# Psy-Fer/SquiggleKit

Measured on AMD Instinct MI355X. Metric: reads/sec MotifSeq DTW (4k-sample read x 200-sample motif), higher is better.
Workload: dtype f64 results; u32 fixed-point screening

## Files before the change

squigglekit_amd/csrc/sk_common.h:

```cpp
#pragma once
#include <hip/hip_runtime.h>
#include <stdint.h>
#include <stddef.h>
#include <stdarg.h>
#include <vector>
#include "squigglekit_hip.h"

#define SK_MAX_DEVICES 16
#define SK_WAVE 64

struct sk_prep {
    int32_t n;
    int32_t flags;
    double  center;
    double  scale;
    double  top;
    double  bot;
};

#define SK_IFLAG_INPLACE 0x100
#define SK_FLAG_PUBLIC   0xff

enum sk_prep_mode { SK_PREP_MEDMAD = 0, SK_PREP_ZSCALE = 1, SK_PREP_SEGMENT = 2, SK_PREP_DRNA = 3 };

// ... 76 lines not shown
    std::vector<int32_t> panel_long;
    sk_buf ckpt;
    sk_buf motifq;
    sk_buf motif64;
    bool   motif64_valid = false;
    std::vector<double> motif64_host;
    sk_buf lastq;
    sk_buf qflag;
    sk_buf wsoft;
    sk_buf lsum;
    sk_buf wstate;
    sk_buf wrec;
    sk_buf wrecq;
    sk_buf order;
    sk_buf motifw;
    std::vector<double> motifw_host;
    int    motifq_L = 0;
    sk_buf retry;
    sk_buf dtwcnt;
    sk_buf audit;
    sk_buf sib;
    sk_buf sibout;
    sk_buf sibstate;
    bool   retry_dev = false;
    std::vector<unsigned> motifq_host;
    bool   motifq_valid = false;
    sk_buf redo;
    int    redo_route = SK_REDO_NONE;
    std::vector<size_t> redo_off;
    size_t redo_used = 0;
    std::vector<int64_t> pa_off_host;
    int    last_retry = 0;
    std::vector<hipEvent_t> evpool;
    int    prof_chunks = 0;
    int    prof_reads[64] = {0};
    std::vector<double> motif_host;
    std::vector<double> motif_src;
    int    motif_L = 0;
    void  *comm = nullptr;
    void  *sessions[SK_STREAM_MAX_SESSIONS] = {};
    sk_buf commbuf;
};

const char *sk_tune(const char *name);

struct sk_entry {
// ... 75 lines not shown
int sk_launch_row_background(sk_ctx *c, const double *rowD, int64_t row_stride, const sk_hit *rec, int32_t nreads,
                             sk_bg_rec *out);
struct sk_path_args {
    int            feed;
    const void    *samples;
    const void    *samples_raw = nullptr;
    int64_t        stride = 0;
    const int64_t *off = nullptr;
    const sk_prep *prep = nullptr;
    int32_t        nreads = 0;
    int64_t        max_len = 0;
    const double  *d_motif = nullptr;
    int32_t        nmotif = 0;
    const sk_hit  *hits = nullptr;
    int32_t        K = 1;
    int32_t       *spans = nullptr;
};
int sk_path_begin(sk_ctx *c);
int sk_launch_paths(sk_ctx *c, const sk_path_args *p);
int sk_launch_events(sk_ctx *c, const sk_path_args *p, sk_event *events);
int sk_launch_events_pool(sk_ctx *c, const sk_event *d_ev, const uint8_t *d_use, int64_t nhits, int32_t N,
                          int32_t *d_idx, int32_t *d_cnt, sk_pool_rec *d_out);
int sk_launch_sdtw_screen(sk_ctx *c, const sk_sdtw_args *a, int ck, int span, int span2,
                          int32_t *d_retry_cnt, int32_t *d_retry, int32_t *d_early_cnt, int32_t *d_early);

__host__ __device__ static inline void sk_slice_indices(int32_t len, int32_t begin, int32_t end, int32_t *lo, int32_t *hi, int *clamped = nullptr)
{
    int64_t s = begin, e = end;
    int cl = 0;
    if (s < 0) { s += len; if (s < 0) { s = 0; cl |= 1; } } else if (s > len) { s = len; cl |= 1; }
    if (e < 0) { e += len; if (e < 0) { e = 0; cl |= 2; } } else if (e > len) { e = len; cl |= 2; }
    *lo = (int32_t)s; *hi = (int32_t)e;
    if (clamped) *clamped = cl;
}
int sk_launch_region_rows_i16(sk_ctx *c, const int16_t *d_sig, int64_t stride, const int32_t *d_len, int32_t nreads,
                              int32_t begin, int32_t end, const int32_t *d_win, int16_t *d_rows, int64_t wstride,
                              int32_t *d_wlen, int32_t *d_from);
int sk_launch_region_rows_f64(sk_ctx *c, const double *d_sig, const int64_t *d_src, const int64_t *d_woff, int32_t nreads,
                              double *d_out);
int sk_panel_plan(sk_ctx *c, const double *motifs, const int32_t *motif_off, int32_t nmotifs, const double *mean,
                  const double *sd, int64_t pairs);
int sk_launch_panel_dtw(sk_ctx *c, const sk_sdtw_args *base, const double *motifs, const int32_t *motif_off,
                        sk_hit *d_all, int64_t out_stride);
int sk_launch_panel_rank(sk_ctx *c, const sk_hit *d_all, int64_t out_stride, int32_t nreads, int32_t nmotifs,
                         sk_panel_rec *d_out);

struct sk_roll_params;
// ... 120 lines not shown
```

squigglekit_amd/csrc/sk_runtime.hip:

```cpp
#include "sk_common.h"
#include <string>
#include <string.h>
#include <mutex>
#include <stdio.h>
#include <stdlib.h>
#include <string.h>

static thread_local char  g_err[512] = "";
static thread_local int   g_cur = -1;
static sk_ctx             g_ctx[SK_MAX_DEVICES];
static std::mutex         g_mu;
static std::recursive_mutex g_ctx_mu[SK_MAX_DEVICES];

int sk_fail(int code, const char *fmt, ...)
{
    va_list ap;
    va_start(ap, fmt);
    vsnprintf(g_err, sizeof g_err, fmt, ap);
    va_end(ap);
    return code;
}

sk_entry::sk_entry() : sk_entry(g_cur) {}

// ... 37 lines not shown
{
    if (!c->stream2) {
        SK_HIP(hipStreamCreateWithFlags(&c->stream2, hipStreamNonBlocking));
        for (int i = 0; i < 9; i++) SK_HIP(hipEventCreateWithFlags(&c->ev_chunk[i], hipEventDisableTiming));
    }
    return SK_OK;
}

struct sk_tunable { const char *name, *test_values, *what; };
static const sk_tunable SK_TUNABLES[] = {
    {"SK_DTW_SCHEME",         "full exact2", "DTW scheme: full = one exact pass, exact2 = two exact passes (default: fixed-point screening + certified window)"},
    {"SK_DTW_QL",             "8 16 64",     "lanes per read of the screening scheme (default: by motif length and batch size)"},
    {"SK_DTW_NOFUSE",         "1",           "filter + medmad as their own kernel instead of the screening pass's prologue"},
    {"SK_DTW_FORCE_RETRY_PM", "100 1000",    "per-mille of reads sent through the exact retry whatever the window pass certified (sensitivity runs)"},
    {"SK_DTW_SPAN",           "150 300",     "look-back of the window pass in columns (one tier)"},
    {"SK_DTW_SPAN2",          "0 500",       "look-back of the window pass's second tier (0: none)"},
    {"SK_DTW_CK",             "64 256",      "steps between checkpoints of the screening pass (multiple of 64)"},
    {"SK_DTW_NOSORT",         "1",           "window passes take the reads in file order"},
    {"SK_DTW_NOHINT",         "1",           "no start hint: the plain screening sweep, every read's exact window looks back the same number of columns"},
    {"SK_DTW_HINT_MIN",       "1",           "the start hint is on for calls of at least this many reads (default 500000)"},
    {"SK_DTW_SORT_MIN",       "1",           "window passes sort chunks of at least this many reads"},
    {"SK_DTW_NO_EARLY",       "1",           "no early exact retry beside the window passes"},
    {"SK_DTW_NO_SIBLINGS",    "1",           "reads whose candidate columns fall into two clusters take the exact pass (no second window)"},
    {"SK_DTW_NOGUARD",        "1",           "screening scheme without its run-time guard (premise test in the window pass, audit, gated exact fallback): A/B cost runs"},
    {"SK_DTW_AUDIT_PERIOD",   "0 1 64",      "the audit re-runs one read in this many with the exact pass (default 4096; 0: no audit)"},
    {"SK_DTW_HOLE",           "qerr1 fma64 fma64x", "tests: a known precision hole put back (E = 1; the fma sample image for float64 reads, with / without the image-error guard) -- the guard has to notice and the records must not change"},
    {"SK_DTW_SCRATCH_MB",     "8 64",        "checkpoint scratch budget in MB (small values force many chunks)"},
    {"SK_DTW_NO_SMALL",       "1",           "small batches keep the batch lane layout"},
    {"SK_DTW_SMALL_MAX",      "0 100000",    "largest batch that spreads a read over 64 lanes"},
    {"SK_PREP_BLOCK",         "1",           "medmad statistics by the workgroup-per-read kernel"},
    {"SK_PREP_ROUNDS",        "1 3",         "grid rounds of the persistent statistics kernels"},
    {"SK_PREP_PERCU",         "1 2",         "workgroups per CU of the persistent statistics kernels"},
    {"SK_SEG_OLD",            "1",           "segmenter: numpy-order statistics kernels for every read"},
    {"SK_SEG_DELTA_SCALE",    "1e13",        "segmenter: certification margin multiplier (large: every read takes the numpy-order redo)"},
    {"SK_SEG_PA_F64",         "1",           "segmenter, raw reads through the pA conversion: expand to float64 and take the float64 kernels instead of the raw-domain kernel"},
    {"SK_SEG_NO_WG",          "1",           "segmenter, reads of 4 097 .. 65 536 samples: the wavefront-per-read statistics kernel (two looks at a read) instead of the workgroup-per-read one"},
    {"SK_SEG_WG_ALL",         "1",           "segmenter: the workgroup-per-read statistics kernel for every row of 4 097 .. 65 536 samples (default: where it is faster)"},
    {"SK_SEG_OCC",            "7 8",         "segmenter statistics kernel: waves per SIMD the registers are sized for"},
    {"SK_SEG_CHUNKS",         "2 8",         "segmenter: chunks of a large batch (walk of one beside the statistics of the next)"},
    {"SK_WALK_GENERAL",       "1",           "segmenter walk: general step (corrector test live)"},
    {"SK_WALK_SYNC",          "1",           "segmenter walk: run hopping with the 64 lanes of a wavefront on the same word (k_seg_walk3)"},
    {"SK_WALK_OWNPASS",       "1",           "segmenter walk: finds the quiet stretches and anchors in a pass of its own instead of taking the statistics kernel's hints"},
    {"SK_WALK_NOJUMP",        "1",           "segmenter walk: every run is hopped through, no jumps between the stretches of quiet entries"},
    {"SK_WALK_NOWAVE",        "1",           "segmenter walk: a lane per read also for long rows / small batches (no wavefront-per-read walk)"},
    {"SK_WALK_WAVE_MAXREADS", "0 1000000",   "segmenter walk: batches of up to this many reads take the wavefront-per-read walk (default: 16384, 131072 for rows beyond 4 096 samples)"},
    {"SK_DRNA_STEP",          "1",           "dRNA_segmenter, both branches: the per-sample scans instead of the scans by runs / by transitions"},
// ... 87 lines not shown
        c->num_cu = prop.multiProcessorCount;
        SK_HIP(hipStreamCreateWithFlags(&c->stream, hipStreamNonBlocking));
        for (int i = 0; i < 4; i++) SK_HIP(hipEventCreate(&c->ev[i]));
        c->ready = true;
    }
    g_cur = slot;
    return SK_OK;
}

static void free_buf(sk_buf *b) { if (b->p) (void)hipFree(b->p); b->p = nullptr; b->cap = 0; }

int sk_shutdown(void)
{
    std::lock_guard<std::mutex> lk(g_mu);
    for (int d = 0; d < SK_MAX_DEVICES; d++) {
        sk_ctx *c = &g_ctx[d];
        std::lock_guard<std::recursive_mutex> c_lock(g_ctx_mu[d]);
        if (!c->ready) continue;
        (void)hipSetDevice(c->device);
        (void)hipStreamSynchronize(c->stream);
        sk_stream_close_all(c);
        sk_buf *bufs[] = {&c->sig, &c->len, &c->off, &c->comp, &c->prep, &c->mask,
                          &c->motif, &c->out, &c->out2, &c->misc, &c->ckpt, &c->retry, &c->motifq, &c->lastq, &c->qflag,
                          &c->motif64, &c->commbuf, &c->dtwcnt, &c->wsoft, &c->wstate, &c->wrec, &c->motifw, &c->lsum, &c->wrecq, &c->order, &c->pacal, &c->seghints, &c->audit, &c->rlen, &c->redo, &c->sib, &c->sibout, &c->sibstate, &c->pull, &c->pulltext, &c->sweep, &c->sweeprec, &c->hitrows, &c->bgrec, &c->pathcnt, &c->pathlist, &c->pathscratch, &c->pathmotif, &c->pathspans, &c->events, &c->poolev, &c->pool, &c->panel, &c->panelwin, &c->panelaux, &c->panelrec, &c->seglev, &c->seglevwork, &c->detect, &c->detectout, &c->hmm, &c->hmmpath, &c->hmmseg};
        for (sk_buf *b : bufs) free_buf(b);
        for (int i = 0; i < 4; i++) (void)hipEventDestroy(c->ev[i]);
        for (hipEvent_t e : c->evpool) (void)hipEventDestroy(e);
        if (c->stream2) {
            (void)hipStreamSynchronize(c->stream2);
            for (int i = 0; i < 9; i++) if (c->ev_chunk[i]) (void)hipEventDestroy(c->ev_chunk[i]);
            (void)hipStreamDestroy(c->stream2);
        }
        if (c->stream3) {
            (void)hipStreamSynchronize(c->stream3);
            for (int i = 0; i < 2; i++) if (c->ev_r[i]) (void)hipEventDestroy(c->ev_r[i]);
            (void)hipStreamDestroy(c->stream3);
        }
        for (int i = 0; i < 2; i++) if (c->ev_s[i]) (void)hipEventDestroy(c->ev_s[i]);
        if (c->stream4) {
            (void)hipStreamSynchronize(c->stream4);
            if (c->ev_a) (void)hipEventDestroy(c->ev_a);
            (void)hipStreamDestroy(c->stream4);
        }
        (void)hipStreamDestroy(c->stream);
        *c = sk_ctx();
    }
    g_cur = -1;
// ... 180 lines not shown
```

squigglekit_amd/csrc/sk_sdtw.hip:

```cpp
#include "sk_sdtw_dev.h"
#include <math.h>
#include <stdlib.h>
#include <string.h>
#include <vector>

namespace {

template <int L, int R, int FEED, int MODE>
__global__ __launch_bounds__(256)
void k_sdtw(const sdtw_kargs a)
{
    static_assert(L == 16 || L == 64, "lanes per read");
    constexpr int G = 64 / L;
    constexpr int SHR = (L == 16) ? DPP_ROW_SHR1 : DPP_WAVE_SHR1;
    constexpr int ROL = (L == 16) ? DPP_ROW_ROL1 : DPP_WAVE_ROL1;
    constexpr bool TRACK = (MODE != MODE_DIST);
    constexpr int CKW = R + 3;
    const double INF = __builtin_huge_val();

    const int lane = threadIdx.x & 63;
    const int wave = blockIdx.x * (blockDim.x >> 6) + (threadIdx.x >> 6);
    const int g = lane / L, l = lane % L;
    int slot = wave * G + g;
    int nreads = a.nreads;
// ... 230 lines not shown
    if (s == 0) { list[0] = naudit; list[1] = 0; }
    if (s >= naudit) return;
    const int64_t base = (int64_t)s * period;
    const int span = (int)min((int64_t)period, (int64_t)nreads - base);
    unsigned h = (unsigned)s * 2654435761u + 0x9E3779B9u;
    h ^= salt * 0x9E3779B9u;
    h ^= h >> 15; h *= 0x85EBCA6Bu; h ^= h >> 13;
    list[2 + s] = (int)(base + (int64_t)(h % (unsigned)span));
}

__global__ void k_audit_compare(const int32_t *list, const sk_hit *exact, sk_hit *out, int naudit, int32_t *guard)
{
    const int s = blockIdx.x * blockDim.x + threadIdx.x;
    if (s >= naudit) return;
    const int r = list[2 + s];
    const sk_hit e = exact[s], g = out[r];
    const bool same_d = (__double_as_longlong(e.dist) == __double_as_longlong(g.dist)) || (e.dist != e.dist && g.dist != g.dist);
    if (same_d && e.start == g.start && e.end == g.end && e.n == g.n) return;
    out[r] = e;
    atomicAdd(&guard[SK_GUARD_MISMATCH], 1);
    atomicAdd(&guard[SK_GUARD_ALARM], 1);
}

static void sk_audit_pick(int32_t *list, int naudit, int period, int nreads, unsigned salt, hipStream_t st)
{
    hipLaunchKernelGGL(k_audit_pick, dim3((naudit + 255) / 256), dim3(256), 0, st, list, naudit, period, nreads, salt);
}
static void sk_audit_compare(const int32_t *list, const sk_hit *exact, sk_hit *out, int naudit, int32_t *guard, hipStream_t st)
{
    hipLaunchKernelGGL(k_audit_compare, dim3((naudit + 255) / 256), dim3(256), 0, st, list, exact, out, naudit, guard);
}

typedef void (*sdtw_fn)(const sdtw_kargs);

template <int L, int FEED, int MODE>
sdtw_fn pick_r(int R)
{
#define SK_KERNEL(RR) k_sdtw<L, RR, FEED, MODE>
    switch (R) { SK_R_CASES_1_16(SK_KERNEL) }
#undef SK_KERNEL
    return nullptr;
}

template <int FEED>
sdtw_fn pick(int L, int R, int mode)
{
// ... 251 lines not shown
    if (const char *e = sk_tune("SK_DTW_SCHEME")) qok = qok && strcmp(e, "exact2") != 0;
    int rc;
    if ((rc = sk_reserve(c, &c->retry, 2 * ((size_t)a->nreads + 2) * sizeof(int32_t)))) return rc;
    if ((rc = sk_reserve(c, &c->dtwcnt, 128))) return rc;
    int32_t *cnt = (int32_t *)c->retry.p;
    int32_t *ecnt = cnt + a->nreads + 2;
    SK_HIP(hipMemsetAsync(cnt, 0, sizeof(int32_t), c->stream));
    SK_HIP(hipMemsetAsync(ecnt, 0, sizeof(int32_t), c->stream));
    if (!a->accumulate) SK_HIP(hipMemsetAsync(c->dtwcnt.p, 0, 128, c->stream));
    c->retry_dev = true;
    if (L == 16 && !c->motif64_valid && pick_any(a->feed, 64, (N + 63) / 64, MODE_FULL)) {
        const int R64 = (N + 63) / 64;
        SK_HIP(hipStreamSynchronize(c->stream));
        if (c->stream3) SK_HIP(hipStreamSynchronize(c->stream3));
        if (c->stream4) SK_HIP(hipStreamSynchronize(c->stream4));
        c->motif64_host.resize((size_t)64 * R64);
        if (!sk_lane_layout(a->motif, N, 64, R64, c->motif64_host.data()))
            return sk_fail(SK_ERR_INVALID, "internal: motif layout mismatch");
        if ((rc = sk_reserve(c, &c->motif64, c->motif64_host.size() * sizeof(double)))) return rc;
        SK_HIP(hipMemcpyAsync(c->motif64.p, c->motif64_host.data(),
                              c->motif64_host.size() * sizeof(double), hipMemcpyHostToDevice, c->stream));
        c->motif64_valid = true;
    }
    auto launch_retry = [&](int32_t *list = nullptr, hipStream_t stream = nullptr) -> int {
        if (!list) list = cnt;
        sdtw_kargs kr = k;
        kr.read0 = 0; kr.ridx = list + 2; kr.count_ptr = list; kr.ckpt = nullptr;
        kr.total_ptr = (int32_t *)c->dtwcnt.p; kr.list_off = 0;
        const int R64 = (N + 63) / 64, P64 = 64 * R64 - N;
        sdtw_fn f64 = (L == 16) ? pick_any(a->feed, 64, R64, MODE_FULL) : nullptr;
        if (f64) {
            sdtw_kargs k64 = kr;
            k64.xlay = (const double *)c->motif64.p; k64.P = P64;
            k64.nreads = a->nreads < 8192 ? a->nreads : 8192;
            int rc2;
            if ((rc2 = launch(c, f64, k64, 64, stream))) return rc2;
            if (a->nreads <= 8192) return SK_OK;
            kr.list_off = 8192; kr.total_ptr = nullptr; kr.nreads = a->nreads - 8192;
            return launch(c, ff, kr, L, stream);
        }
        kr.nreads = a->nreads;
        return launch(c, ff, kr, L, stream);
    };
    if (a->fuse && !qok) return sk_fail(SK_ERR_INVALID, "internal: fused prologue without a screening pass");
    int32_t *guard = (int32_t *)c->dtwcnt.p + 8;
    const bool guarded = qok && sk_tune("SK_DTW_NOGUARD") == nullptr;
    int audit_period = 4096;
    if (const char *e = sk_tune("SK_DTW_AUDIT_PERIOD")) { const int v = atoi(e); if (v >= 0) audit_period = v; }
    int naudit = (guarded && audit_period > 0) ? (int)((a->nreads + audit_period - 1) / audit_period) : 0;
    if (naudit && sk_tune("SK_DTW_AUDIT_PERIOD") == nullptr) {
        const double audit_ms = (double)(maxlen + 64) * (8.0 * ((N + 63) / 64) + 20.0) * 5.0 / 2.4e6;
        const double window_ms = (double)a->nreads * N * 5.85e-8;
        const double call_ms = (double)a->nreads * (double)maxlen * N * 7.4e-11;
        const double exposed = audit_ms - window_ms;
        if (exposed > 0.02 * call_ms) {
            double kd = exposed / (0.02 * call_ms + 1e-9);
            const uint32_t K = kd > 64.0 ? 64u : (uint32_t)kd + 1u;
            if (c->dtw_sparse_calls++ % K) naudit = 0;
        }
    }
    int32_t *alist = nullptr;  sk_hit *aout = nullptr;
    if (naudit) {
        if ((rc = sk_reserve(c, &c->audit, ((size_t)naudit + 2) * sizeof(int32_t) + 16 + (size_t)naudit * sizeof(sk_hit)))) return rc;
        alist = (int32_t *)c->audit.p;
// ... 22 lines not shown
        return launch(c, ff, kr, L, stream);
    };
    auto finish_guard = [&]() -> int {
        if (!guarded) return SK_OK;
        if (naudit) {
            sk_audit_compare(alist, aout, a->out, naudit, guard, c->stream);
            SK_HIP(hipGetLastError());
        }
        sdtw_kargs kf = k;
        kf.read0 = 0; kf.nreads = a->nreads; kf.ridx = nullptr; kf.count_ptr = nullptr; kf.ckpt = nullptr;
        kf.gate_ptr = guard + SK_GUARD_ALARM; kf.guard = guard;
        return launch(c, ff, kf, L);
    };
    if (qok) {
        const bool early = sk_tune("SK_DTW_NO_EARLY") == nullptr;
        if (early && !c->stream3) {
            SK_HIP(hipStreamCreateWithFlags(&c->stream3, hipStreamNonBlocking));
            for (int i = 0; i < 2; i++) SK_HIP(hipEventCreateWithFlags(&c->ev_r[i], hipEventDisableTiming));
        }
        if (early && naudit && !c->stream4) {
            SK_HIP(hipStreamCreateWithFlags(&c->stream4, hipStreamNonBlocking));
            SK_HIP(hipEventCreateWithFlags(&c->ev_a, hipEventDisableTiming));
        }
        if ((rc = sk_launch_sdtw_screen(c, a, ck, span_q, span2, cnt, cnt + 2, early ? ecnt : nullptr,
                                        early ? ecnt + 2 : nullptr))) return rc;
        if (early) {
            SK_HIP(hipStreamWaitEvent(c->stream3, c->ev_r[0], 0));
            if ((rc = launch_retry(ecnt, c->stream3))) return rc;
            SK_HIP(hipEventRecord(c->ev_r[1], c->stream3));
            if (naudit) {
                SK_HIP(hipStreamWaitEvent(c->stream4, c->ev_r[0], 0));
                if ((rc = launch_audit(c->stream4))) return rc;
                SK_HIP(hipEventRecord(c->ev_a, c->stream4));
            }
        }
        if ((rc = launch_retry())) return rc;
        if (early) {
            SK_HIP(hipStreamWaitEvent(c->stream, c->ev_r[1], 0));
            if (naudit) SK_HIP(hipStreamWaitEvent(c->stream, c->ev_a, 0));
        } else if ((rc = launch_audit(nullptr))) return rc;
        if ((rc = finish_guard())) return rc;
        SK_HIP(hipEventRecord(c->ev[3], c->stream));
        return SK_OK;
    }
    const int nck = (int)((maxlen + L - 1) / ck);
    const size_t per_read = (size_t)(nck > 0 ? nck : 1) * L * (R + 3) * sizeof(double);
    int64_t chunk;
    while (true) {
        chunk = sk_dtw_chunk_reads(per_read, a->nreads);
        rc = sk_reserve(c, &c->ckpt, (size_t)chunk * per_read);
        if (rc != SK_ERR_NOMEM || chunk <= 1024) break;
        sk_dtw_scratch_shrink(0);
    }
    if (rc) return rc;
    k.ckpt = (double *)c->ckpt.p; k.nck = nck; k.ck = ck; k.span = span;
    k.retry = cnt + 2; k.retry_cnt = cnt;
    const size_t nchunks = (size_t)((a->nreads + chunk - 1) / chunk);
    while (c->evpool.size() < 3 * nchunks) {
        hipEvent_t e;
        SK_HIP(hipEventCreate(&e));
        c->evpool.push_back(e);
// ... 19 lines not shown
```

squigglekit_amd/csrc/sk_sdtwq.hip:

```cpp
#include "sk_sdtw_dev.h"
#include "sk_prepw_dev.h"
#include <math.h>
#include <stdlib.h>
#include <string.h>
#include <vector>

#ifndef SK_SDTWQ_FEED
#define SK_SDTWQ_FEED 0
#define SK_SDTWQ_MAIN 1
#endif

namespace {

template <int R>
__device__ __forceinline__ void qcolumn(const unsigned (&old)[R], unsigned (&nw)[R], const unsigned (&xq)[R],
                                        unsigned yq, unsigned dg, unsigned up)
{
    constexpr int R4 = R & ~3;
#pragma unroll
    for (int k = 0; k < R4; k += 4) {
        asm("v_min3_u32 %0, %12, %4, %13\n\t"
            "v_sad_u32 %0, %8, %14, %0 clamp\n\t"
            "v_min3_u32 %1, %4, %5, %0\n\t"
            "v_sad_u32 %1, %9, %14, %1 clamp\n\t"
// ... 368 lines not shown
            }
        }
        int tx = 0;
        if constexpr (HINT) {
            tx = max(0, jlo - a.span);
            if (live && bq < QSAFE && jhi >= jlo && jhi - jlo <= a.wmax && sjhi < sjlo) {
                const int hs = hint_start<L>(a, r, bq, l, jlo, jhi);
                if (hs <= jlo) tx = min(max(hs - HINT_MARGIN, 0), max(jlo - 1, 0));
            }
        }
        if (live && l == 0) {
            wrec w;
            w.tbase = tx; w.jlo = jlo; w.jhi = jhi; w.flags = (sjhi >= sjlo) ? 4 : 0;
            ((wrec *)a.wrec_q)[r - a.read0] = w;
            const bool screened = (bq < QSAFE) && (jhi >= jlo) && (jhi - jlo <= a.wmax);
            if (a.early_cnt && n > 0 && !screened) a.early[atomicAdd(a.early_cnt, 1)] = r;
        }
    }
    if (timer && lane == 0) {
        a.clk[0] = __builtin_amdgcn_s_memtime() - tc0;
        a.clk[1] = __builtin_amdgcn_s_memrealtime() - tr0;
    }
}

template <int L, int R, int FEED>
__global__ __launch_bounds__(256)
void SK_P_KERNEL(const sdtw_kargs a)
{
    constexpr int G = 64 / L;
    constexpr int CKW = R + 2;

    const int lane = threadIdx.x & 63;
    const int wave = blockIdx.x * (blockDim.x >> 6) + (threadIdx.x >> 6);
    const int g = lane / L, l = lane % L;
    int slot = wave * G + g;
    int nreads = a.nreads;
    if (a.wl_count) {
        nreads = min(*a.wl_count, a.nreads);
        if (a.total_ptr && blockIdx.x == 0 && threadIdx.x == 0) atomicAdd(a.total_ptr, nreads);
        if (nreads <= 0) return;
    }
    const bool live = slot < nreads;
    if (!live) slot = nreads - 1;
    const int r = a.tier2 == 2 ? ((const sibrec *)a.sib)[slot].r : a.wl_list ? a.wl_list[slot] : a.read0 + slot;

    int n;
    double center = 0.0, scale = 1.0;
    const int16_t *s16 = nullptr;
    const double  *s64 = nullptr;
    if constexpr (FEED == SK_FEED_I16) {
        const sk_prep pr = a.prep[r];
        n = pr.n; center = pr.center; scale = pr.scale;
        s16 = (const int16_t *)a.samples + (int64_t)r * a.stride;
    } else if constexpr (FEED == SK_FEED_F64_NORM) {
        const sk_prep pr = a.prep[r];
        n = pr.n; center = pr.center; scale = pr.scale;
        s64 = (const double *)(((pr.flags & SK_IFLAG_INPLACE) && a.samples_raw) ? a.samples_raw : a.samples) + a.off[r];
    } else {
        n = (int)(a.off[r + 1] - a.off[r]);
        s64 = (const double *)a.samples + a.off[r];
    }
    if (!live) n = 0;

    const unsigned b = (unsigned)a.qflag[r - a.read0];
// ... 85 lines not shown
                qstep(Qs, Qn, y0);
                qstep(Qn, Qs, y1);
            }
            Fq = Fnext;
        }
    }
    if (c0 > 0 && npre == 0) load_ckpt();
    tbase += npre * L;

    if (live) {
        if (c0 > 0) {
            unsigned *ws = a.wstate + ((int64_t)slot * L + l) * CKW;
#pragma unroll
            for (int k = 0; k < R; k++) ws[k] = Qs[k];
            ws[R] = botq; ws[R + 1] = diagq;
        }
        if (l == 0) {
            wrec w;
            w.tbase = tbase; w.jlo = jlo; w.jhi = jhi;
            w.flags = (screened ? 1 : 0) | (c0 > 0 ? 2 : 0) | clustered;
            ((wrec *)a.wrec)[slot] = w;
        }
    }
}

template <int L, int R, int FEED>
__global__ __launch_bounds__(256) __attribute__((amdgpu_waves_per_eu(R <= 13 ? 4 : (R <= 26 ? 3 : 2), 8)))
void k_sdtw_w(const sdtw_kargs a)
{
    constexpr int G = 64 / L;
    constexpr bool XLDS = R > 16;
    constexpr int SHR = (L == 64) ? DPP_WAVE_SHR1 : DPP_ROW_SHR1;
    constexpr int CKW = R + 2;
    constexpr int U = (L < 16) ? L : 8;
    const double INF = __builtin_huge_val();

    const int lane = threadIdx.x & 63;
    const int wave = blockIdx.x * (blockDim.x >> 6) + (threadIdx.x >> 6);
    const int g = lane / L, l = lane % L;
    int slot = wave * G + g;
    int nreads = a.nreads;
    if (a.wl_count) {
        nreads = min(*a.wl_count, a.nreads);
        if (nreads <= 0) return;
    }
    const bool live = slot < nreads;
    if (!live) slot = nreads - 1;
    const int r = a.tier2 == 2 ? ((const sibrec *)a.sib)[slot].r : a.wl_list ? a.wl_list[slot] : a.read0 + slot;

    int n, flags = 0;
    double center = 0.0, scale = 1.0;
    const int16_t *s16 = nullptr;
    const double  *s64 = nullptr;
    if constexpr (FEED == SK_FEED_I16) {
        const sk_prep pr = a.prep[r];
        n = pr.n; flags = pr.flags & SK_FLAG_PUBLIC; center = pr.center; scale = pr.scale;
        s16 = (const int16_t *)a.samples + (int64_t)r * a.stride;
    } else if constexpr (FEED == SK_FEED_F64_NORM) {
        const sk_prep pr = a.prep[r];
        n = pr.n; flags = pr.flags & SK_FLAG_PUBLIC; center = pr.center; scale = pr.scale;
        s64 = (const double *)(((pr.flags & SK_IFLAG_INPLACE) && a.samples_raw) ? a.samples_raw : a.samples) + a.off[r];
    } else {
        n = (int)(a.off[r + 1] - a.off[r]);
        if (n == 0) flags = SK_FLAG_EMPTY;
        s64 = (const double *)a.samples + a.off[r];
    }
    if (!live) n = 0;

// ... 142 lines not shown
        sk_hit h;
        h.n = n; h.flags = flags;
        const bool forced = a.force_retry && (((unsigned)r * 2654435761u) >> 22) < (unsigned)a.force_retry;
        bool certified = false;
        if (a.tier2 == 2) {
            h.dist = best; h.start = bestS; h.end = bestJ;
            h.n = (n > 0 && screened && bestS >= 0 && !forced && premise_holds(best, bestJ)) ? 1 : 0;
            a.sib_out[slot] = h;
        } else if (n <= 0) {
            h.dist = __builtin_nan(""); h.start = -1; h.end = -1;
            a.out[r] = h;
        } else if (screened && bestS >= 0 && !forced && (certified = premise_holds(best, bestJ))) {
            h.dist = best; h.start = bestS; h.end = bestJ;
            a.out[r] = h;
        } else if (!screened && a.early_cnt && !a.tier2) {
        } else {
            h.dist = __builtin_nan(""); h.start = -1; h.end = -1;
            a.out[r] = h;
            const bool violated = screened && bestS >= 0 && !forced && !certified;
            if (screened && a.soft && !forced && !violated) a.soft[atomicAdd(a.soft_cnt, 1)] = r;
            else                                            a.retry[atomicAdd(a.retry_cnt, 1)] = r;
        }
    }
}

typedef void (*sdtw_fn)(const sdtw_kargs);

template <int L, int FEED, int WHICH>
sdtw_fn pick_r(int R)
{
#ifndef SK_SDTWQ_HINT
#define SK_KERNEL(RR) (WHICH == 0 ? (sdtw_fn)SK_Q_KERNEL<L, RR, FEED, false> :     \
                       WHICH == 3 ? (sdtw_fn)SK_Q_KERNEL<L, RR, FEED, (RR >= 2)> : \
                       WHICH == 1 ? (sdtw_fn)SK_P_KERNEL<L, RR, FEED> : (sdtw_fn)k_sdtw_w<L, RR, FEED>)
#else
#define SK_KERNEL(RR) (WHICH == 0 ? (sdtw_fn)SK_Q_KERNEL<L, RR, FEED, false> :     \
                       WHICH == 3 ? (sdtw_fn)SK_Q_KERNEL<L, RR, FEED, (RR >= 2)> : (sdtw_fn)SK_P_KERNEL<L, RR, FEED>)
#endif
    switch (R) { SK_R_CASES_1_16(SK_KERNEL) }
    if constexpr (L != 64) {
        switch (R) { SK_R_CASES_17_32(SK_KERNEL) }
    }
#undef SK_KERNEL
    return nullptr;
}

template <int WHICH, int FEED>
sdtw_fn pick_l(int L, int R)
{
    if (L == 8)  return pick_r<8, FEED, WHICH>(R);
    if (L == 16) return pick_r<16, FEED, WHICH>(R);
#ifndef SK_SDTWQ_HINT
    return pick_r<64, FEED, WHICH>(R);
#else
    return nullptr;
#endif
}

}

#if defined(SK_SDTWQ_HINT)
void *sk_sdtwq_pick_hint(int which, int L, int R)
#elif SK_SDTWQ_FEED == 0
void *sk_sdtwq_pick_feed0(int which, int L, int R)
#elif SK_SDTWQ_FEED == 1
void *sk_sdtwq_pick_feed1(int which, int L, int R)
#else
void *sk_sdtwq_pick_feed2(int which, int L, int R)
#endif
{
    switch (which) {
    case 0: return (void *)pick_l<0, SK_SDTWQ_FEED>(L, R);
    case 1: return (void *)pick_l<1, SK_SDTWQ_FEED>(L, R);
    case 3: return (void *)pick_l<3, SK_SDTWQ_FEED>(L, R);
#ifndef SK_SDTWQ_HINT
    default: return (void *)pick_l<2, SK_SDTWQ_FEED>(L, R);
#else
    default: return nullptr;
#endif
    }
}

#ifdef SK_SDTWQ_MAIN
void *sk_sdtwq_pick_feed1(int which, int L, int R);
void *sk_sdtwq_pick_feed2(int which, int L, int R);
void *sk_sdtwq_pick_hint(int which, int L, int R);

static void screen_layout(int N, int64_t nreads, int64_t maxlen, int *L, int *R)
{
    int l = (N <= 8 * 32 && nreads >= (maxlen > 8192 ? 65536 : 49152)) ? 8 : (N <= 16 * 32) ? 16 : 64;
    if (const char *e = sk_tune("SK_DTW_QL")) {
        const int v = atoi(e);
        if ((v == 8 && N <= 8 * 32) || (v == 16 && N <= 16 * 32) || v == 64) l = v;
    }
    *L = l;
    *R = (N + l - 1) / l;
}

// ... 58 lines not shown
__global__ __launch_bounds__(ORDER_TPB) void k_order_scatter(const order_args a)
{
    __shared__ int h[ORDER_BINS];
    for (int b = threadIdx.x; b < ORDER_BINS; b += ORDER_TPB) h[b] = 0;
    __syncthreads();
    int key[ORDER_IPT], rank[ORDER_IPT];
#pragma unroll
    for (int u = 0; u < ORDER_IPT; u++) {
        const int i = (blockIdx.x * ORDER_IPT + u) * ORDER_TPB + threadIdx.x;
        key[u] = 0; rank[u] = 0;
        if (i < a.nreads) { key[u] = order_key(a, i); rank[u] = atomicAdd(&h[key[u]], 1); }
    }
    __syncthreads();
    for (int b = threadIdx.x; b < ORDER_BINS; b += ORDER_TPB)
        if (h[b]) h[b] = atomicAdd(&a.hist[b], h[b]);
    __syncthreads();
#pragma unroll
    for (int u = 0; u < ORDER_IPT; u++) {
        const int i = (blockIdx.x * ORDER_IPT + u) * ORDER_TPB + threadIdx.x;
        if (i < a.nreads) a.order[h[key[u]] + rank[u]] = a.read0 + i;
    }
}

__global__ void k_sib_combine(const sibrec *sib, const int32_t *cnt, int cap, const sk_hit *so, sk_hit *out,
                              int32_t *retry, int32_t *retry_cnt, int32_t *nsib_total)
{
    const int s = blockIdx.x * blockDim.x + threadIdx.x;
    if (s == 0 && nsib_total) atomicAdd(nsib_total, min(*cnt, cap));
    if (s >= min(*cnt, cap)) return;
    const int r = sib[s].r;
    sk_hit A = out[r];
    const sk_hit B = so[s];
    if (A.start < 0) return;
    if (B.n == 1) {
        if (B.dist < A.dist) { A.dist = B.dist; A.start = B.start; A.end = B.end; out[r] = A; }
    } else {
        A.dist = __builtin_nan(""); A.start = -1; A.end = -1;
        out[r] = A;
        retry[atomicAdd(retry_cnt, 1)] = r;
    }
}

int sk_launch_sdtw_screen(sk_ctx *c, const sk_sdtw_args *a, int ck, int span, int span2,
                          int32_t *d_retry_cnt, int32_t *d_retry, int32_t *d_early_cnt, int32_t *d_early)
{
    const int N = a->nmotif;
    int L, R;
    screen_layout(N, a->nreads, a->max_len, &L, &R);
    const int P = L * R - N;
    int rc;
    if (!c->motifq_valid || c->motifq_L != L) {
        SK_HIP(hipStreamSynchronize(c->stream));
        std::vector<unsigned> &layq = c->motifq_host;
        std::vector<double> &layw = c->motifw_host;
        layq.resize((size_t)L * R);
        layw.resize((size_t)L * R);
        if (!sk_lane_layout(a->motif, N, L, R, layw.data())) return sk_fail(SK_ERR_INVALID, "internal: motif layout mismatch");
        for (size_t i = 0; i < layw.size(); i++)
            layq[i] = (unsigned)((int)rint(layw[i] * QSCALE)) + 0x80000000u;
        if ((rc = sk_reserve(c, &c->motifq, layq.size() * sizeof(unsigned)))) return rc;
        if ((rc = sk_reserve(c, &c->motifw, layw.size() * sizeof(double)))) return rc;
        SK_HIP(hipMemcpyAsync(c->motifq.p, layq.data(), layq.size() * sizeof(unsigned), hipMemcpyHostToDevice, c->stream));
        SK_HIP(hipMemcpyAsync(c->motifw.p, layw.data(), layw.size() * sizeof(double), hipMemcpyHostToDevice, c->stream));
        c->motifq_valid = true;
        c->motifq_L = L;
    }

// ... 25 lines not shown
    const bool tiers = span2 > span;
    if (tiers && (rc = sk_reserve(c, &c->wsoft, ((size_t)chunk + 1) * sizeof(int32_t)))) return rc;
    const bool siblings = sk_tune("SK_DTW_NO_SIBLINGS") == nullptr;
    const int sib_cap = (int)(chunk / 64 + 1024);
    if (siblings) {
        if ((rc = sk_reserve(c, &c->sib, 16 + (size_t)sib_cap * sizeof(sibrec)))) return rc;
        if ((rc = sk_reserve(c, &c->sibout, (size_t)sib_cap * sizeof(sk_hit)))) return rc;
        if ((rc = sk_reserve(c, &c->sibstate, (size_t)sib_cap * (state_bytes + sizeof(wrec))))) return rc;
        if (c->stream3 && !c->ev_s[0])
            for (int i = 0; i < 2; i++) SK_HIP(hipEventCreateWithFlags(&c->ev_s[i], hipEventDisableTiming));
    }

    typedef void *(*pick_fn)(int, int, int);
    const pick_fn pk = a->feed == SK_FEED_I16 ? (pick_fn)sk_sdtwq_pick_feed0
                     : a->feed == SK_FEED_F64_NORM ? (pick_fn)sk_sdtwq_pick_feed1 : (pick_fn)sk_sdtwq_pick_feed2;
    sdtw_fn fq = (sdtw_fn)pk(P == 0 ? 3 : 0, L, R), fp = (sdtw_fn)pk(1, L, R), fw = (sdtw_fn)pk(2, L, R);
    const int64_t plen = (int64_t)N + maxlen + 2;
    int64_t hint_min = HINT_MIN_READS;
    if (const char *e = sk_tune("SK_DTW_HINT_MIN")) { const int v = atoi(e); if (v > 0) hint_min = v; }
    const bool hint = a->feed == SK_FEED_I16 && (L == 8 || L == 16) && plen <= HINT_MAX_PLEN && R <= HINT_MAX_R &&
                      N >= HINT_MIN_N && a->nreads >= hint_min && sk_tune("SK_DTW_NOHINT") == nullptr;
    sdtw_fn fp1 = fp;
    if (hint) { fq = (sdtw_fn)sk_sdtwq_pick_hint(P == 0 ? 3 : 0, L, R); fp1 = (sdtw_fn)sk_sdtwq_pick_hint(1, L, R); }
    if (!fq || !fp || !fp1 || !fw) return sk_fail(SK_ERR_UNSUPPORTED, "no screening kernel for L=%d R=%d", L, R);

    sdtw_kargs k = kargs_of(a);
    k.xlay = (const double *)c->motifw.p; k.xlayq = (const unsigned *)c->motifq.p; k.P = P; k.out = a->out;
    k.nck = nck; k.ck = ck; k.span = span; k.retry = d_retry; k.retry_cnt = d_retry_cnt;
    k.ckq = (unsigned *)c->ckpt.p; k.lastq = (unsigned *)c->lastq.p; k.lq_stride = (int64_t)lq_stride;
    k.qflag = (int32_t *)c->qflag.p; k.lsum = (unsigned *)c->lsum.p;
    k.wstate = (unsigned *)c->wstate.p; k.wrec = c->wrec.p; k.wrec_q = c->wrecq.p;
    k.early_cnt = d_early_cnt; k.early = d_early;
    k.qplen = (unsigned)plen;
    k.qerr = hint ? ((unsigned)plen << HINT_T) + HINT_MASK : (unsigned)plen;
    k.wmax = 4 * ck;
    k.lds_wave_words = (64 / L) * ck;
    k.guard = sk_tune("SK_DTW_NOGUARD") ? nullptr : (int32_t *)c->dtwcnt.p + 8;
    k.wsteps = (unsigned long long *)((char *)c->dtwcnt.p + 64);
    if (const char *e = sk_tune("SK_DTW_HOLE")) {
        k.hole = strcmp(e, "qerr1") == 0 ? SK_HOLE_QERR1 : strcmp(e, "fma64") == 0 ? SK_HOLE_FMA64
               : strcmp(e, "fma64x") == 0 ? SK_HOLE_FMA64_UNGUARDED : SK_HOLE_NONE;
        if (k.hole == SK_HOLE_QERR1) k.qerr = 1;
    }
    if (const char *e = sk_tune("SK_DTW_FORCE_RETRY_PM")) {
        const int pm = atoi(e);
        if (pm > 0) k.force_retry = pm >= 1000 ? 1024 : (pm * 1024 + 999) / 1000;
    }
// ... 25 lines not shown
            k.fz_raw = fz.raw; k.fz_len = fz.len; k.fz_lo = fz.lo; k.fz_hi = fz.hi;
            k.fz_mode = fz.mode == SK_PREP_ZSCALE ? 1 : 0;
            k.fz_vec = ((((uintptr_t)fz.raw & 15) == 0 && (a->stride % 8) == 0) ? 1 : 0) |
                       ((((uintptr_t)a->samples & 15) == 0 && (a->stride % 8) == 0) ? 2 : 0);
        }
        hipEvent_t *ev = &c->evpool[3 * (size_t)c->prof_chunks];
        k.sib = nullptr; k.sib_cnt = nullptr; k.sib_out = nullptr; k.tier2 = 0;
        if (siblings) {
            SK_HIP(hipMemsetAsync(c->sib.p, 0, 16, c->stream));
            k.sib_cnt = (int32_t *)c->sib.p; k.sib = (char *)c->sib.p + 16; k.sib_out = (sk_hit *)c->sibout.p;
            k.sib_cap = sib_cap;
        }
        SK_HIP(hipEventRecord(ev[0], c->stream));
        k.clk = (r0 == 0) ? (unsigned long long *)((char *)c->dtwcnt.p + 16) : nullptr;
        hipLaunchKernelGGL(fq, dim3(grid), dim3(256), fz_lds, c->stream, k);
        k.fz_raw = nullptr;
        if (d_early_cnt && r0 + chunk >= a->nreads) SK_HIP(hipEventRecord(c->ev_r[0], c->stream));
        SK_HIP(hipGetLastError());
        if (siblings) {
            sdtw_kargs ks = k;
            ks.tier2 = 2; ks.wl_list = nullptr; ks.wl_count = k.sib_cnt; ks.soft = nullptr; ks.soft_cnt = nullptr;
            ks.span = tiers ? span2 : span; ks.total_ptr = nullptr; ks.nreads = sib_cap;
            ks.wstate = (unsigned *)c->sibstate.p; ks.wrec = (char *)c->sibstate.p + (size_t)sib_cap * state_bytes;
            const int sgrid = (sib_cap + reads_per_block - 1) / reads_per_block;
            hipStream_t ss = c->stream3 ? c->stream3 : c->stream;
            if (c->stream3) {
                SK_HIP(hipEventRecord(c->ev_s[0], c->stream));
                SK_HIP(hipStreamWaitEvent(c->stream3, c->ev_s[0], 0));
            }
            hipLaunchKernelGGL(fp, dim3(sgrid), dim3(256), 0, ss, ks);
            hipLaunchKernelGGL(fw, dim3(sgrid), dim3(256), 0, ss, ks);
            SK_HIP(hipGetLastError());
            if (c->stream3) SK_HIP(hipEventRecord(c->ev_s[1], c->stream3));
        }
        SK_HIP(hipEventRecord(ev[1], c->stream));
        const int32_t *order = nullptr;
        if (sorted && k.nreads >= sort_min) {
            order_args oa;
            oa.rec = (const wrec *)c->wrecq.p; oa.qflag = (const int32_t *)c->qflag.p;
            oa.nreads = k.nreads; oa.read0 = k.read0; oa.span = span; oa.ck = ck; oa.nck = nck; oa.L = L; oa.wmax = k.wmax;
            oa.hint = hint ? 1 : 0;
            oa.hist = (int32_t *)c->order.p; oa.order = oa.hist + ORDER_BINS;
            SK_HIP(hipMemsetAsync(oa.hist, 0, ORDER_BINS * sizeof(int32_t), c->stream));
            const int og = (k.nreads + ORDER_TPB * ORDER_IPT - 1) / (ORDER_TPB * ORDER_IPT);
            hipLaunchKernelGGL(k_order_count, dim3(og), dim3(ORDER_TPB), 0, c->stream, oa);
            hipLaunchKernelGGL(k_order_scan, dim3(1), dim3(ORDER_BINS), 0, c->stream, oa.hist);
            hipLaunchKernelGGL(k_order_scatter, dim3(og), dim3(ORDER_TPB), 0, c->stream, oa);
            SK_HIP(hipGetLastError());
            order = oa.order;
        }
        k.tier2 = 0;
        if (tiers) {
            int32_t *soft = (int32_t *)c->wsoft.p;
            SK_HIP(hipMemsetAsync(soft, 0, sizeof(int32_t), c->stream));
            k.span = span; k.wl_list = order; k.wl_count = nullptr; k.soft = soft + 1; k.soft_cnt = soft;
            hipLaunchKernelGGL(fp1, dim3(grid), dim3(256), 0, c->stream, k);
            hipLaunchKernelGGL(fw, dim3(grid), dim3(256), 0, c->stream, k);
            SK_HIP(hipGetLastError());
            k.span = span2; k.wl_list = soft + 1; k.wl_count = soft; k.soft = nullptr; k.soft_cnt = nullptr;
            k.tier2 = 1;
            k.total_ptr = (int32_t *)c->dtwcnt.p + 1;
        } else {
            k.wl_list = order; k.wl_count = nullptr;
        }
        hipLaunchKernelGGL(tiers ? fp : fp1, dim3(grid), dim3(256), 0, c->stream, k);
        k.total_ptr = nullptr;
        hipLaunchKernelGGL(fw, dim3(grid), dim3(256), 0, c->stream, k);
        SK_HIP(hipGetLastError());
        if (siblings) {
            if (c->stream3) SK_HIP(hipStreamWaitEvent(c->stream, c->ev_s[1], 0));
            hipLaunchKernelGGL(k_sib_combine, dim3((sib_cap + 255) / 256), dim3(256), 0, c->stream,
                               (const sibrec *)k.sib, (const int32_t *)k.sib_cnt, sib_cap, (const sk_hit *)k.sib_out, k.out,
                               d_retry, d_retry_cnt, (int32_t *)c->dtwcnt.p + 8 + 6);
            SK_HIP(hipGetLastError());
        }
        SK_HIP(hipEventRecord(ev[2], c->stream));
        c->prof_reads[c->prof_chunks < 64 ? c->prof_chunks : 63] = k.nreads;
        c->prof_chunks++;
    }
    return SK_OK;
}
#endif
```

Baseline: 17.41 million.

## Walk short window-pass lists with capped persistent grids; retry failed siblings early

Adds grid-stride 'list walking' variants of the window-pass kernels, used for the second-tier and sibling-cluster rounds so launches over short device-side lists use a capped grid (default 1024 workgroups) instead of one sized for the whole chunk. Sibling reads whose second window fails are collected by a new kernel into a list that gets the exact retry early on the side stream, and their results are merged by slot. This aims to cut the cost of launching and exiting many empty workgroups and to take sibling failures off the main retry path. It adds extra kernels, buffers and cross-stream bookkeeping, and the capped grid may underuse the GPU when the lists are long.

```diff
diff --git a/squigglekit_amd/csrc/sk_common.h b/squigglekit_amd/csrc/sk_common.h
--- a/squigglekit_amd/csrc/sk_common.h
+++ b/squigglekit_amd/csrc/sk_common.h
@@ -122,6 +122,7 @@
     sk_buf sib;
     sk_buf sibout;
     sk_buf sibstate;
+    sk_buf sibx;
     bool   retry_dev = false;
     std::vector<unsigned> motifq_host;
     bool   motifq_valid = false;
@@ -243,7 +244,8 @@
 int sk_launch_events_pool(sk_ctx *c, const sk_event *d_ev, const uint8_t *d_use, int64_t nhits, int32_t N,
                           int32_t *d_idx, int32_t *d_cnt, sk_pool_rec *d_out);
 int sk_launch_sdtw_screen(sk_ctx *c, const sk_sdtw_args *a, int ck, int span, int span2,
-                          int32_t *d_retry_cnt, int32_t *d_retry, int32_t *d_early_cnt, int32_t *d_early);
+                          int32_t *d_retry_cnt, int32_t *d_retry, int32_t *d_early_cnt, int32_t *d_early,
+                          int32_t *d_sfail, int sfail_cap);
 
 __host__ __device__ static inline void sk_slice_indices(int32_t len, int32_t begin, int32_t end, int32_t *lo, int32_t *hi, int *clamped = nullptr)
 {
diff --git a/squigglekit_amd/csrc/sk_runtime.hip b/squigglekit_amd/csrc/sk_runtime.hip
--- a/squigglekit_amd/csrc/sk_runtime.hip
+++ b/squigglekit_amd/csrc/sk_runtime.hip
@@ -83,6 +83,7 @@
     {"SK_DTW_SORT_MIN",       "1",           "window passes sort chunks of at least this many reads"},
     {"SK_DTW_NO_EARLY",       "1",           "no early exact retry beside the window passes"},
     {"SK_DTW_NO_SIBLINGS",    "1",           "reads whose candidate columns fall into two clusters take the exact pass (no second window)"},
+    {"SK_DTW_TIER_GRID",      "0 1",         "workgroups of the window-pass rounds over a short list (second tier, second clusters; default 1024; 1: one workgroup walks the whole list; 0: launches sized for the chunk)"},
     {"SK_DTW_NOGUARD",        "1",           "screening scheme without its run-time guard (premise test in the window pass, audit, gated exact fallback): A/B cost runs"},
     {"SK_DTW_AUDIT_PERIOD",   "0 1 64",      "the audit re-runs one read in this many with the exact pass (default 4096; 0: no audit)"},
     {"SK_DTW_HOLE",           "qerr1 fma64 fma64x", "tests: a known precision hole put back (E = 1; the fma sample image for float64 reads, with / without the image-error guard) -- the guard has to notice and the records must not change"},
@@ -216,7 +217,7 @@
         sk_stream_close_all(c);
         sk_buf *bufs[] = {&c->sig, &c->len, &c->off, &c->comp, &c->prep, &c->mask,
                           &c->motif, &c->out, &c->out2, &c->misc, &c->ckpt, &c->retry, &c->motifq, &c->lastq, &c->qflag,
-                          &c->motif64, &c->commbuf, &c->dtwcnt, &c->wsoft, &c->wstate, &c->wrec, &c->motifw, &c->lsum, &c->wrecq, &c->order, &c->pacal, &c->seghints, &c->audit, &c->rlen, &c->redo, &c->sib, &c->sibout, &c->sibstate, &c->pull, &c->pulltext, &c->sweep, &c->sweeprec, &c->hitrows, &c->bgrec, &c->pathcnt, &c->pathlist, &c->pathscratch, &c->pathmotif, &c->pathspans, &c->events, &c->poolev, &c->pool, &c->panel, &c->panelwin, &c->panelaux, &c->panelrec, &c->seglev, &c->seglevwork, &c->detect, &c->detectout, &c->hmm, &c->hmmpath, &c->hmmseg};
+                          &c->motif64, &c->commbuf, &c->dtwcnt, &c->wsoft, &c->wstate, &c->wrec, &c->motifw, &c->lsum, &c->wrecq, &c->order, &c->pacal, &c->seghints, &c->audit, &c->rlen, &c->redo, &c->sib, &c->sibout, &c->sibstate, &c->sibx, &c->pull, &c->pulltext, &c->sweep, &c->sweeprec, &c->hitrows, &c->bgrec, &c->pathcnt, &c->pathlist, &c->pathscratch, &c->pathmotif, &c->pathspans, &c->events, &c->poolev, &c->pool, &c->panel, &c->panelwin, &c->panelaux, &c->panelrec, &c->seglev, &c->seglevwork, &c->detect, &c->detectout, &c->hmm, &c->hmmpath, &c->hmmseg};
         for (sk_buf *b : bufs) free_buf(b);
         for (int i = 0; i < 4; i++) (void)hipEventDestroy(c->ev[i]);
         for (hipEvent_t e : c->evpool) (void)hipEventDestroy(e);
diff --git a/squigglekit_amd/csrc/sk_sdtw.hip b/squigglekit_amd/csrc/sk_sdtw.hip
--- a/squigglekit_amd/csrc/sk_sdtw.hip
+++ b/squigglekit_amd/csrc/sk_sdtw.hip
@@ -276,6 +276,12 @@
     atomicAdd(&guard[SK_GUARD_ALARM], 1);
 }
 
+__global__ void k_exact_merge(const int32_t *list, int cap, const sk_hit *recs, sk_hit *out)
+{
+    const int s = blockIdx.x * blockDim.x + threadIdx.x;
+    if (s < min(list[0], cap)) out[list[2 + s]] = recs[s];
+}
+
 static void sk_audit_pick(int32_t *list, int naudit, int period, int nreads, unsigned salt, hipStream_t st)
 {
     hipLaunchKernelGGL(k_audit_pick, dim3((naudit + 255) / 256), dim3(256), 0, st, list, naudit, period, nreads, salt);
@@ -573,24 +579,26 @@
                               c->motif64_host.size() * sizeof(double), hipMemcpyHostToDevice, c->stream));
         c->motif64_valid = true;
     }
-    auto launch_retry = [&](int32_t *list = nullptr, hipStream_t stream = nullptr) -> int {
+    auto launch_retry = [&](int32_t *list = nullptr, hipStream_t stream = nullptr, int cap = 0, sk_hit *by_slot = nullptr) -> int {
         if (!list) list = cnt;
+        if (cap <= 0) cap = a->nreads;
         sdtw_kargs kr = k;
         kr.read0 = 0; kr.ridx = list + 2; kr.count_ptr = list; kr.ckpt = nullptr;
         kr.total_ptr = (int32_t *)c->dtwcnt.p; kr.list_off = 0;
+        if (by_slot) { kr.out = by_slot; kr.out_by_slot = 1; }
         const int R64 = (N + 63) / 64, P64 = 64 * R64 - N;
         sdtw_fn f64 = (L == 16) ? pick_any(a->feed, 64, R64, MODE_FULL) : nullptr;
         if (f64) {
             sdtw_kargs k64 = kr;
             k64.xlay = (const double *)c->motif64.p; k64.P = P64;
-            k64.nreads = a->nreads < 8192 ? a->nreads : 8192;
+            k64.nreads = cap < 8192 ? cap : 8192;
             int rc2;
             if ((rc2 = launch(c, f64, k64, 64, stream))) return rc2;
-            if (a->nreads <= 8192) return SK_OK;
-            kr.list_off = 8192; kr.total_ptr = nullptr; kr.nreads = a->nreads - 8192;
+            if (cap <= 8192) return SK_OK;
+            kr.list_off = 8192; kr.total_ptr = nullptr; kr.nreads = cap - 8192;
             return launch(c, ff, kr, L, stream);
         }
-        kr.nreads = a->nreads;
+        kr.nreads = cap;
         return launch(c, ff, kr, L, stream);
     };
     if (a->fuse && !qok) return sk_fail(SK_ERR_INVALID, "internal: fused prologue without a screening pass");
@@ -659,10 +667,20 @@
             SK_HIP(hipStreamCreateWithFlags(&c->stream4, hipStreamNonBlocking));
             SK_HIP(hipEventCreateWithFlags(&c->ev_a, hipEventDisableTiming));
         }
+        const int sfail_cap = (int)(a->nreads / 64 + 1024);
+        int32_t *sfail = nullptr;  sk_hit *sfail_out = nullptr;
+        if (early) {
+            const size_t list_bytes = (((size_t)sfail_cap + 2) * sizeof(int32_t) + 15) & ~(size_t)15;
+            if ((rc = sk_reserve(c, &c->sibx, list_bytes + (size_t)sfail_cap * sizeof(sk_hit)))) return rc;
+            sfail = (int32_t *)c->sibx.p;
+            sfail_out = (sk_hit *)((char *)c->sibx.p + list_bytes);
+            SK_HIP(hipMemsetAsync(sfail, 0, sizeof(int32_t), c->stream));
+        }
         if ((rc = sk_launch_sdtw_screen(c, a, ck, span_q, span2, cnt, cnt + 2, early ? ecnt : nullptr,
-                                        early ? ecnt + 2 : nullptr))) return rc;
+                                        early ? ecnt + 2 : nullptr, sfail, sfail_cap))) return rc;
         if (early) {
             SK_HIP(hipStreamWaitEvent(c->stream3, c->ev_r[0], 0));
+            if ((rc = launch_retry(sfail, c->stream3, sfail_cap, sfail_out))) return rc;
             if ((rc = launch_retry(ecnt, c->stream3))) return rc;
             SK_HIP(hipEventRecord(c->ev_r[1], c->stream3));
             if (naudit) {
@@ -674,6 +692,9 @@
         if ((rc = launch_retry())) return rc;
         if (early) {
             SK_HIP(hipStreamWaitEvent(c->stream, c->ev_r[1], 0));
+            hipLaunchKernelGGL(k_exact_merge, dim3((sfail_cap + 255) / 256), dim3(256), 0, c->stream,
+                               (const int32_t *)sfail, sfail_cap, (const sk_hit *)sfail_out, a->out);
+            SK_HIP(hipGetLastError());
             if (naudit) SK_HIP(hipStreamWaitEvent(c->stream, c->ev_a, 0));
         } else if ((rc = launch_audit(nullptr))) return rc;
         if ((rc = finish_guard())) return rc;
diff --git a/squigglekit_amd/csrc/sk_sdtwq.hip b/squigglekit_amd/csrc/sk_sdtwq.hip
--- a/squigglekit_amd/csrc/sk_sdtwq.hip
+++ b/squigglekit_amd/csrc/sk_sdtwq.hip
@@ -1,3 +1,4 @@
+#ifndef SK_SDTWQ_WALK
 #include "sk_sdtw_dev.h"
 #include "sk_prepw_dev.h"
 #include <math.h>
@@ -414,24 +415,43 @@
         a.clk[1] = __builtin_amdgcn_s_memrealtime() - tr0;
     }
 }
-
+#endif
+
+#ifdef SK_SDTWQ_WALK
+#undef SK_P_KERNEL
+#define SK_P_KERNEL k_sdtw_pl
+#define SK_W_KERNEL k_sdtw_wl
+#define SK_BLOCK wg
+#else
+#define SK_W_KERNEL k_sdtw_w
+#define SK_BLOCK blockIdx.x
+#endif
 template <int L, int R, int FEED>
 __global__ __launch_bounds__(256)
 void SK_P_KERNEL(const sdtw_kargs a)
 {
     constexpr int G = 64 / L;
     constexpr int CKW = R + 2;
+#ifdef SK_SDTWQ_WALK
+    const int nlist = min(*a.wl_count, a.nreads);
+    if (a.total_ptr && blockIdx.x == 0 && threadIdx.x == 0) atomicAdd(a.total_ptr, nlist);
+    for (int wg = blockIdx.x; (int64_t)wg * (4 * G) < nlist; wg += gridDim.x) {
+#endif
 
     const int lane = threadIdx.x & 63;
-    const int wave = blockIdx.x * (blockDim.x >> 6) + (threadIdx.x >> 6);
+    const int wave = SK_BLOCK * (blockDim.x >> 6) + (threadIdx.x >> 6);
     const int g = lane / L, l = lane % L;
     int slot = wave * G + g;
+#ifdef SK_SDTWQ_WALK
+    const int nreads = nlist;
+#else
     int nreads = a.nreads;
     if (a.wl_count) {
         nreads = min(*a.wl_count, a.nreads);
         if (a.total_ptr && blockIdx.x == 0 && threadIdx.x == 0) atomicAdd(a.total_ptr, nreads);
         if (nreads <= 0) return;
     }
+#endif
     const bool live = slot < nreads;
     if (!live) slot = nreads - 1;
     const int r = a.tier2 == 2 ? ((const sibrec *)a.sib)[slot].r : a.wl_list ? a.wl_list[slot] : a.read0 + slot;
@@ -563,11 +583,18 @@
             ((wrec *)a.wrec)[slot] = w;
         }
     }
+#ifdef SK_SDTWQ_WALK
+    }
+#endif
 }
 
 template <int L, int R, int FEED>
+#ifdef SK_SDTWQ_WALK
+__global__ __launch_bounds__(256)
+#else
 __global__ __launch_bounds__(256) __attribute__((amdgpu_waves_per_eu(R <= 13 ? 4 : (R <= 26 ? 3 : 2), 8)))
-void k_sdtw_w(const sdtw_kargs a)
+#endif
+void SK_W_KERNEL(const sdtw_kargs a)
 {
     constexpr int G = 64 / L;
     constexpr bool XLDS = R > 16;
@@ -575,16 +602,24 @@
     constexpr int CKW = R + 2;
     constexpr int U = (L < 16) ? L : 8;
     const double INF = __builtin_huge_val();
+#ifdef SK_SDTWQ_WALK
+    const int nlist = min(*a.wl_count, a.nreads);
+    for (int wg = blockIdx.x; (int64_t)wg * (4 * G) < nlist; wg += gridDim.x) {
+#endif
 
     const int lane = threadIdx.x & 63;
-    const int wave = blockIdx.x * (blockDim.x >> 6) + (threadIdx.x >> 6);
+    const int wave = SK_BLOCK * (blockDim.x >> 6) + (threadIdx.x >> 6);
     const int g = lane / L, l = lane % L;
     int slot = wave * G + g;
+#ifdef SK_SDTWQ_WALK
+    const int nreads = nlist;
+#else
     int nreads = a.nreads;
     if (a.wl_count) {
         nreads = min(*a.wl_count, a.nreads);
         if (nreads <= 0) return;
     }
+#endif
     const bool live = slot < nreads;
     if (!live) slot = nreads - 1;
     const int r = a.tier2 == 2 ? ((const sibrec *)a.sib)[slot].r : a.wl_list ? a.wl_list[slot] : a.read0 + slot;
@@ -773,7 +808,22 @@
             else                                            a.retry[atomicAdd(a.retry_cnt, 1)] = r;
         }
     }
-}
+#ifdef SK_SDTWQ_WALK
+    __syncthreads();
+    }
+#endif
+}
+#undef SK_W_KERNEL
+#undef SK_BLOCK
+
+#ifndef SK_SDTWQ_WALK
+#ifndef SK_SDTWQ_HINT
+#define SK_SDTWQ_WALK
+#include "sk_sdtwq.hip"
+#undef SK_SDTWQ_WALK
+#undef SK_P_KERNEL
+#define SK_P_KERNEL k_sdtw_p
+#endif
 
 typedef void (*sdtw_fn)(const sdtw_kargs);
 
@@ -783,7 +833,8 @@
 #ifndef SK_SDTWQ_HINT
 #define SK_KERNEL(RR) (WHICH == 0 ? (sdtw_fn)SK_Q_KERNEL<L, RR, FEED, false> :     \
                        WHICH == 3 ? (sdtw_fn)SK_Q_KERNEL<L, RR, FEED, (RR >= 2)> : \
-                       WHICH == 1 ? (sdtw_fn)SK_P_KERNEL<L, RR, FEED> : (sdtw_fn)k_sdtw_w<L, RR, FEED>)
+                       WHICH == 1 ? (sdtw_fn)SK_P_KERNEL<L, RR, FEED> : WHICH == 2 ? (sdtw_fn)k_sdtw_w<L, RR, FEED> : \
+                       WHICH == 4 ? (sdtw_fn)k_sdtw_pl<L, RR, FEED> : (sdtw_fn)k_sdtw_wl<L, RR, FEED>)
 #else
 #define SK_KERNEL(RR) (WHICH == 0 ? (sdtw_fn)SK_Q_KERNEL<L, RR, FEED, false> :     \
                        WHICH == 3 ? (sdtw_fn)SK_Q_KERNEL<L, RR, FEED, (RR >= 2)> : (sdtw_fn)SK_P_KERNEL<L, RR, FEED>)
@@ -825,6 +876,8 @@
     case 1: return (void *)pick_l<1, SK_SDTWQ_FEED>(L, R);
     case 3: return (void *)pick_l<3, SK_SDTWQ_FEED>(L, R);
 #ifndef SK_SDTWQ_HINT
+    case 4: return (void *)pick_l<4, SK_SDTWQ_FEED>(L, R);
+    case 5: return (void *)pick_l<5, SK_SDTWQ_FEED>(L, R);
     default: return (void *)pick_l<2, SK_SDTWQ_FEED>(L, R);
 #else
     default: return nullptr;
@@ -929,8 +982,17 @@
     }
 }
 
+__global__ void k_sib_failed(const sibrec *sib, const int32_t *cnt, int cap, sk_hit *so, int32_t *list, int lcap)
+{
+    const int s = blockIdx.x * blockDim.x + threadIdx.x;
+    if (s >= min(*cnt, cap) || so[s].n != 0) return;
+    const int idx = atomicAdd(list, 1);
+    if (idx < lcap) { list[2 + idx] = sib[s].r; so[s].n = -1; }
+    else            atomicSub(list, 1);
+}
+
 __global__ void k_sib_combine(const sibrec *sib, const int32_t *cnt, int cap, const sk_hit *so, sk_hit *out,
-                              int32_t *retry, int32_t *retry_cnt, int32_t *nsib_total)
+                              int32_t *retry, int32_t *retry_cnt, int32_t *retried, int32_t *nsib_total)
 {
     const int s = blockIdx.x * blockDim.x + threadIdx.x;
     if (s == 0 && nsib_total) atomicAdd(nsib_total, min(*cnt, cap));
@@ -938,6 +1000,12 @@
     const int r = sib[s].r;
     sk_hit A = out[r];
     const sk_hit B = so[s];
+    if (B.n == -1) {
+        if (A.start < 0) atomicSub(retried, 1);
+        A.dist = __builtin_nan(""); A.start = -1; A.end = -1;
+        out[r] = A;
+        return;
+    }
     if (A.start < 0) return;
     if (B.n == 1) {
         if (B.dist < A.dist) { A.dist = B.dist; A.start = B.start; A.end = B.end; out[r] = A; }
@@ -949,7 +1017,8 @@
 }
 
 int sk_launch_sdtw_screen(sk_ctx *c, const sk_sdtw_args *a, int ck, int span, int span2,
-                          int32_t *d_retry_cnt, int32_t *d_retry, int32_t *d_early_cnt, int32_t *d_early)
+                          int32_t *d_retry_cnt, int32_t *d_retry, int32_t *d_early_cnt, int32_t *d_early,
+                          int32_t *d_sfail, int sfail_cap)
 {
     const int N = a->nmotif;
     int L, R;
@@ -1021,7 +1090,10 @@
                       N >= HINT_MIN_N && a->nreads >= hint_min && sk_tune("SK_DTW_NOHINT") == nullptr;
     sdtw_fn fp1 = fp;
     if (hint) { fq = (sdtw_fn)sk_sdtwq_pick_hint(P == 0 ? 3 : 0, L, R); fp1 = (sdtw_fn)sk_sdtwq_pick_hint(1, L, R); }
-    if (!fq || !fp || !fp1 || !fw) return sk_fail(SK_ERR_UNSUPPORTED, "no screening kernel for L=%d R=%d", L, R);
+    int tier_grid = 1024;
+    if (const char *e = sk_tune("SK_DTW_TIER_GRID")) { const int v = atoi(e); if (v >= 0) tier_grid = v; }
+    const sdtw_fn fpl = tier_grid ? (sdtw_fn)pk(4, L, R) : fp, fwl = tier_grid ? (sdtw_fn)pk(5, L, R) : fw;
+    if (!fq || !fp || !fp1 || !fw || !fpl || !fwl) return sk_fail(SK_ERR_UNSUPPORTED, "no screening kernel for L=%d R=%d", L, R);
 
     sdtw_kargs k = kargs_of(a);
     k.xlay = (const double *)c->motifw.p; k.xlayq = (const unsigned *)c->motifq.p; k.P = P; k.out = a->out;
@@ -1093,14 +1165,18 @@
             ks.tier2 = 2; ks.wl_list = nullptr; ks.wl_count = k.sib_cnt; ks.soft = nullptr; ks.soft_cnt = nullptr;
             ks.span = tiers ? span2 : span; ks.total_ptr = nullptr; ks.nreads = sib_cap;
             ks.wstate = (unsigned *)c->sibstate.p; ks.wrec = (char *)c->sibstate.p + (size_t)sib_cap * state_bytes;
-            const int sgrid = (sib_cap + reads_per_block - 1) / reads_per_block;
+            int sgrid = (sib_cap + reads_per_block - 1) / reads_per_block;
+            if (tier_grid && sgrid > tier_grid) sgrid = tier_grid;
             hipStream_t ss = c->stream3 ? c->stream3 : c->stream;
             if (c->stream3) {
                 SK_HIP(hipEventRecord(c->ev_s[0], c->stream));
                 SK_HIP(hipStreamWaitEvent(c->stream3, c->ev_s[0], 0));
             }
-            hipLaunchKernelGGL(fp, dim3(sgrid), dim3(256), 0, ss, ks);
-            hipLaunchKernelGGL(fw, dim3(sgrid), dim3(256), 0, ss, ks);
+            hipLaunchKernelGGL(fpl, dim3(sgrid), dim3(256), 0, ss, ks);
+            hipLaunchKernelGGL(fwl, dim3(sgrid), dim3(256), 0, ss, ks);
+            if (d_sfail && c->stream3)
+                hipLaunchKernelGGL(k_sib_failed, dim3((sib_cap + 255) / 256), dim3(256), 0, ss, (const sibrec *)ks.sib,
+                                   (const int32_t *)ks.sib_cnt, sib_cap, ks.sib_out, d_sfail, sfail_cap);
             SK_HIP(hipGetLastError());
             if (c->stream3) SK_HIP(hipEventRecord(c->ev_s[1], c->stream3));
         }
@@ -1134,15 +1210,16 @@
         } else {
             k.wl_list = order; k.wl_count = nullptr;
         }
-        hipLaunchKernelGGL(tiers ? fp : fp1, dim3(grid), dim3(256), 0, c->stream, k);
+        const int grid2 = (tiers && tier_grid && grid > tier_grid) ? tier_grid : grid;
+        hipLaunchKernelGGL(tiers ? fpl : fp1, dim3(grid2), dim3(256), 0, c->stream, k);
         k.total_ptr = nullptr;
-        hipLaunchKernelGGL(fw, dim3(grid), dim3(256), 0, c->stream, k);
+        hipLaunchKernelGGL(tiers ? fwl : fw, dim3(grid2), dim3(256), 0, c->stream, k);
         SK_HIP(hipGetLastError());
         if (siblings) {
             if (c->stream3) SK_HIP(hipStreamWaitEvent(c->stream, c->ev_s[1], 0));
             hipLaunchKernelGGL(k_sib_combine, dim3((sib_cap + 255) / 256), dim3(256), 0, c->stream,
                                (const sibrec *)k.sib, (const int32_t *)k.sib_cnt, sib_cap, (const sk_hit *)k.sib_out, k.out,
-                               d_retry, d_retry_cnt, (int32_t *)c->dtwcnt.p + 8 + 6);
+                               d_retry, d_retry_cnt, (int32_t *)c->dtwcnt.p, (int32_t *)c->dtwcnt.p + 8 + 6);
             SK_HIP(hipGetLastError());
         }
         SK_HIP(hipEventRecord(ev[2], c->stream));
@@ -1152,3 +1229,4 @@
     return SK_OK;
 }
 #endif
+#endif
```

Result: no change. 17.40 million (median of 2 runs) (-0.1%).
